# kserve/modelmesh

Hardware: AMD Instinct MI355X
Metric: placement decisions/sec at 100k models x 10k pods; p99 decision latency (higher is better)
Workload: dtype i64; 1 GPU; C3: 100000 models x 10000 pods, 8 load-target decision(s) per model per step = 800000 decisions per launch (SURVEY.md §8d synthetic fleet); streams=4, hw_queues=4, distinct_batches=6, issuers=1, library_submission_threads=0, resident_input_bytes=384000000

## Files before the change

modelmesh_amd/csrc/mmplace.hip:

```cpp
#include <hip/hip_runtime.h>
#include <dlfcn.h>
#include <rccl/rccl.h>
#include <rocprim/device/device_radix_sort.hpp>
#include <chrono>
#include <rocprim/device/device_merge_sort.hpp>
#include <rocprim/device/device_scan.hpp>

#include <algorithm>
#include <atomic>
#include <cstdarg>
#include <cstdio>
#include <cstdlib>
#include <cstring>
#include <map>
#include <memory>
#include <mutex>
#include <shared_mutex>
#include <thread>
#include <new>
#include <string>
#include <unordered_map>
#include <vector>

#include "../../include/mmplace.h"
// ... 21 lines not shown
    void *p = nullptr;
    size_t cap = 0;
    hipError_t ensure(size_t bytes)
    {
        if (bytes <= cap) return hipSuccess;
        if (p) (void)hipFree(p);
        p = nullptr;
        cap = 0;
        size_t want = std::max<size_t>(bytes, 256);
        want = (want + 255) & ~size_t(255);
        hipError_t e = hipMalloc(&p, want);
        if (e == hipSuccess) cap = want;
        return e;
    }
    void release()
    {
        if (p) (void)hipFree(p);
        p = nullptr;
        cap = 0;
    }
    template <class T>
    T *as() const { return reinterpret_cast<T *>(p); }
};

struct SnapBufs {
    DevBuf pods, lru, rem, cnt, rpm, orig, pos_of, elig, elig_nors, pref, has_pref, fullw, ge, pc, ph, nz, heads, bslots, bpm, bwin, bsurv, bpcs;
    DevBuf sel, rk;
    DevBuf amul;
    int32_t amul_w = 0;
    DevBuf memo, memo_cand, memo_rk;
    DevBuf lmemo;
    DevBuf ctpos;
    uint64_t types_gen = 0;
    int32_t n_bslots = 0;
    void release()
    {
        for (DevBuf *b : {&pods, &lru, &rem, &cnt, &rpm, &orig, &pos_of, &elig, &elig_nors, &pref, &has_pref, &fullw, &ge, &pc, &ph, &nz, &heads, &bslots, &bpm, &bwin, &bsurv, &bpcs, &ctpos, &sel, &rk, &amul, &memo, &memo_cand, &memo_rk, &lmemo})
            b->release();
    }
};

template <class SnapT>
SnapT snap_columns(const SnapBufs &B, int32_t P, int32_t W, int32_t T, bool any_rs, int64_t min_space)
{
    SnapT S{};
    S.P = P;
    S.W = W;
    S.T = T;
    S.any_rs = any_rs;
    S.min_space = min_space;
    S.lru = B.lru.as<int64_t>();
    S.rem = B.rem.as<int64_t>();
    S.cnt = B.cnt.as<int32_t>();
    S.rpm = B.rpm.as<int32_t>();
    S.orig = B.orig.as<int32_t>();
    S.pos_of = B.pos_of.as<int32_t>();
    S.elig = B.elig.as<uint64_t>();
    S.elig_nors = B.elig_nors.as<uint64_t>();
    S.pref = B.pref.as<uint64_t>();
    S.has_pref = B.has_pref.as<uint8_t>();
    S.fullw = B.fullw.as<uint64_t>();
    return S;
}

struct SnapSide {
    DevBuf d_allowed, d_has_allowed, stats_acc, d_pts, d_prohib, pstats, tstats, rmodels;
    DevBuf mtw;
    uint64_t types_gen = 0;
    bool rmodels_ok = false;
    std::vector<int32_t> pts_of;
    std::vector<uint64_t> pts_prohib;
    int32_t n_pts = 0, pts_tw = 1;
    std::vector<StatsAcc> pstats_h, tstats_h;
    void release()
    {
        for (DevBuf *b : {&d_allowed, &d_has_allowed, &stats_acc, &d_pts, &d_prohib, &pstats, &tstats, &rmodels, &mtw}) b->release();
    }
};

}

constexpr unsigned int kPinnedFlags = hipHostMallocCoherent | hipHostMallocMapped;
constexpr size_t kSelMaxBytes = (size_t)32 << 20;
constexpr int kTailStaticLds = 512;
constexpr int kTailBlocks = 16;
constexpr int kMaxMissBufs = 64;
constexpr int kFastSlots = 4;
constexpr int kFastN = 4096;
constexpr int kFastExtra = 16384;
struct FastSlot {
    std::mutex mu;
    hipStream_t stream = nullptr;
    mmp_place_req *reqs = nullptr;
    int32_t *extra = nullptr;
    mmp_place_out *outs = nullptr;
    uint32_t *done = nullptr;
    uint32_t *blocks = nullptr;
    std::atomic<uint32_t> seq{0};
};

struct Tuning {
    int32_t force_wave = 0;
    int32_t no_memo = 0;
    int32_t memo_from = -1;
    int32_t no_long_memo = 0;
    int32_t no_split = 0;
    int32_t split_from = -1;
    int32_t tail_blocks = kTailBlocks;
    int32_t split_notail = 0;
    int32_t no_long_lds = 0;
    int32_t no_caseb = 0;
    int32_t long_dense_from = kLongDenseFrom;
    bool long_dense_env = false;
    int32_t long_mode = -1;
    int32_t rank_mode = 0;
    int32_t no_delta = 0;
    int32_t plan_sorted = 0;
    int32_t plan_fused = 1;
    int32_t resident = 0;
};

struct mmp_ctx {
    mmp_config cfg{};
    hipStream_t stream = nullptr;
    std::mutex batch_mu, err_mu, cs_mu;
    std::shared_mutex mu;
    std::shared_ptr<struct IssuePool> pool;
    std::mutex pool_mu;
    struct Resident {
        std::atomic<bool> enabled{false}, running{false};
        std::atomic<uint32_t> generation{0};
        hipStream_t stream = nullptr;
        ResidentSlot *slots = nullptr;
        ResidentAnswer *answers = nullptr;
        ResidentCtl *ctl = nullptr;
        std::mutex launch_mu;
        std::mutex slot_mu[kResidentSlots];
        uint32_t seq[kResidentSlots] = {};
        std::atomic<uint32_t> rr{0};
        long long idle_ticks = 5'000'000;
        std::atomic<uint64_t> launches{0}, served{0}, punted{0};
        std::atomic<int> slow{0};
        std::atomic<int> punt_streak{0}, skip{0};
    } res;
    std::vector<hipStream_t> caller_streams;
    std::string err;
    FastSlot fast[kFastSlots];
    std::atomic<uint32_t> fast_rr{0};
    bool prof = false, prof_armed = false;
    hipEvent_t pe0 = nullptr, pe1 = nullptr;
    double last_kernel_ms = -1.0;
    size_t lds_limit = 64 * 1024;
    DevBuf rt_sreqs, rt_souts, rt_cnt;
    hipEvent_t reg_event = nullptr;
    std::atomic<bool> reg_pending{false};
    std::atomic<size_t> lds_granted{48 * 1024};
    Tuning tune;
    int32_t plan_grid_max = 0;
    struct MissBuf {
        std::mutex mu;
        bool used = false;
        hipStream_t st = nullptr;
        int32_t *words = nullptr;
        size_t cap = 0;
        int32_t *report = nullptr;
    };
    MissBuf miss_bufs[kMaxMissBufs];
// ... 348 lines not shown
    A.extra = static_cast<const int32_t *>(d_extra);
    A.outs = static_cast<mmp_place_out *>(d_outs);
    A.n = n;
    A.n_models = c->n_models;
    A.now = now;
    A.n_pods_all = n_pods_all;
    return A;
}

struct PlaceCall {
    const mmp_place_caller *caller = nullptr;
    int32_t extra_bound = 0;
    uint32_t *done_flag = nullptr;
    uint32_t done_seq = 0;
    uint32_t *done_blocks = nullptr;
    const mmp_place_req *inline_req = nullptr;
    const PlaceSegs *segs = nullptr;
    int32_t seg_blocks = 0;
    const GateArgs *fused_gate = nullptr;
    const mmp_gate_req *fused_greq = nullptr;
};

PlaceCall slot_call(FastSlot *f, const mmp_place_req *inline_req)
{
    PlaceCall o;
    o.done_flag = f->done;
    o.done_seq = ++f->seq;
    o.done_blocks = f->blocks;
    o.inline_req = inline_req;
    return o;
}

enum class PlaceRoute {
    memo_split, memo_split_c,
    multi, multi_m, multi_long, multi_long4,
    miss_single, single_lean, flag,
    batch, batch_m, batch_c, batch_c_m, batch_long, batch_long4, batch_long_c, batch_long4_c,
};
bool is_split(PlaceRoute r) { return r == PlaceRoute::memo_split || r == PlaceRoute::memo_split_c; }

struct RouteState {
    bool snap_long = false, snap_full = false;
    bool memo = false, lmemo = false;
    bool wins = false, rmodels = false;
    bool split_ok = false;
    bool memo_tail_lds = false;
};

bool long_first(const RouteState &s) { return s.snap_long && s.snap_full && s.rmodels; }

int32_t dense_from(const Tuning &t, const RouteState &s)
{
    return (long_first(s) && s.lmemo && !t.long_dense_env) ? INT32_MAX : t.long_dense_from;
}

PlaceRoute place_route(const Tuning &t, const RouteState &s, int32_t n, const PlaceCall &o)
{
    const bool caller = o.caller != nullptr, latency = o.inline_req || o.done_flag;
    const bool use_memo = !latency && !s.snap_long && !t.no_memo && !t.force_wave && s.wins && s.rmodels && s.memo &&
                          n >= (t.memo_from >= 0 ? t.memo_from : (caller ? kMemoFromC : kMemoFrom));
    const bool split = !o.segs && !t.no_split && s.split_ok;
    if (use_memo && split && s.memo_tail_lds && n >= (t.split_from >= 0 ? t.split_from : (caller ? kSplitFromC : kSplitFrom)))
        return caller ? PlaceRoute::memo_split_c : PlaceRoute::memo_split;
    if (o.segs) {
        if (s.snap_long) return n >= t.long_dense_from ? PlaceRoute::multi_long4 : PlaceRoute::multi_long;
        return use_memo ? PlaceRoute::multi_m : PlaceRoute::multi;
    }
    if (o.inline_req) return o.fused_gate ? PlaceRoute::miss_single : PlaceRoute::single_lean;
    if (o.done_flag && n > kPlaceBlock) return PlaceRoute::flag;
    if (caller && s.snap_long) return n >= dense_from(t, s) ? PlaceRoute::batch_long4_c : PlaceRoute::batch_long_c;
    if (use_memo) return caller ? PlaceRoute::batch_c_m : PlaceRoute::batch_m;
    if (caller) return PlaceRoute::batch_c;
    if (s.snap_long) return n >= dense_from(t, s) ? PlaceRoute::batch_long4 : PlaceRoute::batch_long;
    return PlaceRoute::batch;
}

template <class K>
const void *kfn(K *k) { return reinterpret_cast<const void *>(k); }
int grant_place_lds(mmp_ctx *c)
{
    static std::mutex grant_mu;
    std::lock_guard<std::mutex> g(grant_mu);
    const int want = (int)(c->lds_limit - kPlaceStaticLds);
    const int tail = want - kTailStaticLds;
    const struct {
        const void *fn;
        int max_lds;
    } kernels[] = {
        {kfn(place_batch_kernel), want}, {kfn(place_batch_m_kernel), want}, {kfn(place_batch_c_kernel), want},
        {kfn(place_batch_c_m_kernel), want}, {kfn(place_batch_long_kernel), want}, {kfn(place_batch_long4_kernel), want},
        {kfn(place_batch_long_c_kernel), want}, {kfn(place_batch_long4_c_kernel), want}, {kfn(place_batch_flag_kernel), want},
        {kfn(place_single_lean_kernel), want}, {kfn(miss_single_kernel), want}, {kfn(place_multi_kernel), want},
        {kfn(place_multi_m_kernel), want}, {kfn(place_multi_long_kernel), want}, {kfn(place_multi_long4_kernel), want},
        {kfn(place_tail_kernel), tail}, {kfn(place_tail_c_kernel), tail},
    };
    for (const auto &k : kernels) HIP_TRY(c, hipFuncSetAttribute(k.fn, hipFuncAttributeMaxDynamicSharedMemorySize, k.max_lds));
    c->lds_granted.store((size_t)want, std::memory_order_release);
    return MMP_OK;
}

int place_launch(mmp_ctx *c, const void *d_reqs, int32_t n, const void *d_extra, int64_t now, void *d_outs, hipStream_t st,
                 const PlaceCall &o = PlaceCall{})
{
    if (n == 0) return MMP_OK;
    if (o.caller && (o.segs || o.inline_req || o.done_flag)) return fail(c, MMP_EINVAL, "the single-caller form takes the batch kernels only");
    const Tuning &t = c->tune;
    const Snap &S = c->snap;
    const SnapBufs &B = c->sb[c->cur];
    PlaceArgs A = place_args(c, d_reqs, n, d_extra, now, d_outs, true, S.P);
    A.mtw = cur_side(c).rmodels_ok ? cur_side(c).mtw.as<int32_t>() : nullptr;
    A.wins = c->n_shards > 0 ? nullptr : B.heads.as<TypeWin>();
    A.force_wave = t.force_wave;
    A.done_flag = o.done_flag;
    A.done_seq = o.done_seq;
    A.extra_bound = o.extra_bound;
    RouteState rs;
    rs.snap_long = c->snap_long, rs.snap_full = c->snap_full, rs.memo = S.memo != nullptr, rs.lmemo = S.lmemo != nullptr;
    rs.wins = A.wins != nullptr, rs.rmodels = A.rmodels != nullptr;
    const bool latency = o.inline_req || o.done_flag;
    const int wpad = (S.W + 1) & ~1;
    size_t lds = std::max<size_t>((size_t)kPlaceWaves * 2 * wpad * sizeof(uint64_t), (size_t)place_lane_lds(S.T));
    A.long_first = long_first(rs) ? 1 : 0;
    if (A.long_first && !latency && !t.no_long_lds && n >= dense_from(t, rs)) {
        const size_t tb = long_tables_bytes(S.T, S.W);
        if (tb <= 24 * 1024 && ((lds + 15) & ~(size_t)15) + tb + kPlaceStaticLds <= c->lds_limit) {
            const size_t off = (lds + 15) & ~(size_t)15;
            A.long_first = 1 + (int32_t)off;
            lds = off + tb;
        }
    }
    if (c->snap_long && !latency && A.wins && !t.no_caseb && B.n_bslots > 0) {
        A.bslots = B.bslots.as<BSlot>();
        A.n_bslots = std::min(B.n_bslots, kBSlots);
        A.bwin = B.bwin.as<BLaunch>();
        A.bsurv = B.bsurv.as<uint64_t>();
        A.bpcs = B.bpcs.as<int32_t>();
    }
    if (lds + kPlaceStaticLds > c->lds_limit)
        return fail(c, MMP_EINVAL, "instance table too large for the LDS staging tile (%d pods: %zu + %d bytes of LDS, the device "
                    "gives a workgroup %zu)", S.P, lds, kPlaceStaticLds, c->lds_limit);
    if (lds > c->lds_granted.load(std::memory_order_acquire))
        if (const int rc = grant_place_lds(c)) return rc;
    const size_t lds_nobar = (size_t)kPlaceWaves * place_wave_lds(wpad);
    rs.memo_tail_lds = lds + kPlaceStaticLds + kTailStaticLds <= c->lds_limit;
    HIP_TRY(c, order_after_registry(c, st));
    const int grid = div_up(n, kPlaceBlock);
    const int cap = rest_list_cap(grid * kPlaceWaves);
    int32_t *words = nullptr, *report = nullptr;
    std::unique_lock<std::mutex> pair;
    rs.split_ok = !c->split_off.load(std::memory_order_relaxed);
    PlaceRoute r = place_route(t, rs, n, o);
    if (is_split(r) && (!miss_buffer(c, st, rest_buffer_ints(grid * kPlaceWaves), &words, &report, pair) ||
                        c->split_off.load(std::memory_order_relaxed))) {
        if (pair) pair.unlock();
        rs.split_ok = false;
        r = place_route(t, rs, n, o);
    }
    if (t.split_notail) words = nullptr;
    const size_t lds_memo = (size_t)kPlaceWaves * memo_stage_bytes(S.T);
    const dim3 block(kPlaceBlock), tails(t.tail_blocks);
    const bool tail = !t.split_notail;
    const mmp_place_caller C = o.caller ? *o.caller : mmp_place_caller{};
    switch (r) {
    case PlaceRoute::memo_split:
        hipLaunchKernelGGL(place_memo_kernel, dim3(grid), block, lds_memo, st, S, A, words, cap);
        if (tail) hipLaunchKernelGGL(place_tail_kernel, tails, block, lds, st, S, A, wpad, words, cap, report);
        break;
    case PlaceRoute::memo_split_c:
        hipLaunchKernelGGL(place_memo_c_kernel, dim3(grid), block, lds_memo, st, S, A, words, cap, C);
        if (tail) hipLaunchKernelGGL(place_tail_c_kernel, tails, block, lds, st, S, A, wpad, words, cap, report, C);
        break;
    case PlaceRoute::multi: hipLaunchKernelGGL(place_multi_kernel, dim3(o.seg_blocks), block, lds, st, S, A, wpad, *o.segs); break;
    case PlaceRoute::multi_m: hipLaunchKernelGGL(place_multi_m_kernel, dim3(o.seg_blocks), block, lds_nobar, st, S, A, wpad, *o.segs); break;
    case PlaceRoute::multi_long: hipLaunchKernelGGL(place_multi_long_kernel, dim3(o.seg_blocks), block, lds, st, S, A, wpad, *o.segs); break;
    case PlaceRoute::multi_long4: hipLaunchKernelGGL(place_multi_long4_kernel, dim3(o.seg_blocks), block, lds, st, S, A, wpad, *o.segs); break;
    case PlaceRoute::miss_single:
        hipLaunchKernelGGL(miss_single_kernel, dim3(1), dim3(128), lds, st, S, A, wpad, *o.inline_req, *o.fused_gate, *o.fused_greq);
        break;
    case PlaceRoute::single_lean: hipLaunchKernelGGL(place_single_lean_kernel, dim3(1), dim3(64), lds, st, S, A, wpad, *o.inline_req); break;
    case PlaceRoute::flag: hipLaunchKernelGGL(place_batch_flag_kernel, dim3(grid), block, lds, st, S, A, wpad, o.done_blocks); break;
    case PlaceRoute::batch: hipLaunchKernelGGL(place_batch_kernel, dim3(grid), block, lds, st, S, A, wpad); break;
    case PlaceRoute::batch_m: hipLaunchKernelGGL(place_batch_m_kernel, dim3(grid), block, lds_nobar, st, S, A, wpad); break;
    case PlaceRoute::batch_c: hipLaunchKernelGGL(place_batch_c_kernel, dim3(grid), block, lds, st, S, A, wpad, C); break;
    case PlaceRoute::batch_c_m: hipLaunchKernelGGL(place_batch_c_m_kernel, dim3(grid), block, lds_nobar, st, S, A, wpad, C); break;
    case PlaceRoute::batch_long: hipLaunchKernelGGL(place_batch_long_kernel, dim3(grid), block, lds_nobar, st, S, A, wpad); break;
    case PlaceRoute::batch_long4: hipLaunchKernelGGL(place_batch_long4_kernel, dim3(grid), block, lds, st, S, A, wpad); break;
    case PlaceRoute::batch_long_c: hipLaunchKernelGGL(place_batch_long_c_kernel, dim3(grid), block, lds_nobar, st, S, A, wpad, C); break;
    case PlaceRoute::batch_long4_c: hipLaunchKernelGGL(place_batch_long4_c_kernel, dim3(grid), block, lds, st, S, A, wpad, C); break;
    }
    HIP_TRY(c, hipGetLastError());
    if (is_split(r)) c->n_split.fetch_add(1, std::memory_order_relaxed);
    return MMP_OK;
}

}

extern "C" {

int mmp_abi_version(void) { return MMP_ABI_VERSION; }

int64_t mmp_min_space_units(int32_t dflt, int32_t threads, int64_t cap_units, int have_unload)
{
    const int32_t mn = (int32_t)((uint32_t)dflt * ((have_unload || threads <= 1) ? 1u : 2u));
    const int32_t a = (int32_t)((uint32_t)dflt * (uint32_t)threads);
    const int32_t b = (int32_t)(cap_units / 20);
    const int32_t target = a < b ? a : b;
    return mn > target ? mn : target;
}

int mmp_create(const mmp_config *cfg, mmp_ctx **out)
{
    if (!cfg || !out) return fail(nullptr, MMP_EINVAL, "mmp_create: null argument");
    *out = nullptr;
    int ndev = 0;
    hipError_t e = hipGetDeviceCount(&ndev);
    if (e != hipSuccess || ndev <= 0)
        return fail(nullptr, MMP_ENODEVICE, "no HIP device available (%s); libmmplace has no CPU path",
                    e == hipSuccess ? "device count 0" : hipGetErrorString(e));
    if (cfg->device < 0 || cfg->device >= ndev)
        return fail(nullptr, MMP_EINVAL, "device %d out of range (have %d)", cfg->device, ndev);
    if ((e = hipSetDevice(cfg->device)) != hipSuccess)
        return fail(nullptr, MMP_EHIP, "hipSetDevice: %s", hipGetErrorString(e));
    mmp_ctx *c = new (std::nothrow) mmp_ctx();
    if (!c) return fail(nullptr, MMP_ENOMEM, "out of memory");
    c->cfg = *cfg;
    {
        int v = 0;
        if (hipDeviceGetAttribute(&v, hipDeviceAttributeMaxSharedMemoryPerBlock, cfg->device) == hipSuccess && v > 0) c->lds_limit = (size_t)v;
    }
    c->tune = read_tuning();
    {
        int cus = 0, per_cu = 0;
        if (hipDeviceGetAttribute(&cus, hipDeviceAttributeMultiprocessorCount, cfg->device) == hipSuccess && cus > 0 &&
            hipFuncSetAttribute(reinterpret_cast<const void *>(proactive_plan_fused_kernel), hipFuncAttributeMaxDynamicSharedMemorySize,
                                (int)kPlanFusedLds) == hipSuccess &&
            hipOccupancyMaxActiveBlocksPerMultiprocessor(&per_cu, proactive_plan_fused_kernel, kPlanFusedBlock, kPlanFusedLds) == hipSuccess &&
            per_cu > 0)
            c->plan_grid_max = std::min(cus, kPlanFusedGrid);
        (void)hipGetLastError();
    }
    if ((e = hipStreamCreateWithFlags(&c->stream, hipStreamNonBlocking)) != hipSuccess) {
        delete c;
        return fail(nullptr, MMP_EHIP, "hipStreamCreate: %s", hipGetErrorString(e));
    }
    if ((e = hipEventCreateWithFlags(&c->reg_event, hipEventDisableTiming)) != hipSuccess) {
        (void)hipStreamDestroy(c->stream);
        delete c;
        return fail(nullptr, MMP_EHIP, "hipEventCreate: %s", hipGetErrorString(e));
    }
    for (FastSlot &f : c->fast) {
        int lo = 0, hi = 0;
        (void)hipDeviceGetStreamPriorityRange(&lo, &hi);
        hipError_t e1 = hipStreamCreateWithPriority(&f.stream, hipStreamNonBlocking, hi);
// ... 3961 lines not shown
```

modelmesh_amd/csrc/place_kernel.hpp:

```cpp
#pragma once
#include "snapshot.hpp"

namespace mmp {

#ifndef MMP_PLACE_WAVES
#define MMP_PLACE_WAVES 4
#endif
constexpr int kPlaceWaves = MMP_PLACE_WAVES;
constexpr int kPlaceBlock = kPlaceWaves * 64;

#ifdef MMP_PHASE_CLOCK
__device__ unsigned int g_phase[4096][16];
#define PHASE_ROW() (((blockIdx.x * (blockDim.x >> 6)) + (threadIdx.x >> 6)) & 4095)
#define PHASE_T0() unsigned long long ph_t_ = __builtin_amdgcn_s_memtime()
#define PHASE(k)                                                                                   \
    do {                                                                                           \
        const unsigned long long t_ = __builtin_amdgcn_s_memtime();                                \
        if (lane_id() == __ffsll((unsigned long long)__ballot(1)) - 1) g_phase[PHASE_ROW()][k] = (unsigned int)(t_ - ph_t_); \
        ph_t_ = t_;                                                                                \
    } while (0)
#define PHASE_COUNT(k, n)                                                                          \
    do {                                                                                           \
        if (lane_id() == __ffsll((unsigned long long)__ballot(1)) - 1) g_phase[PHASE_ROW()][k] += (unsigned int)(n); \
    } while (0)
// ... 2392 lines not shown
            const int rho_s = null_s ? 1 + srk - g0 : 0;
            bool self_pending = null_s;
            int t = index + (null0 ? 1 : 0);
#pragma unroll
            for (int i = 0; i < kInlineExcl; i++) {
                if (self_pending && selfpos < sx[i]) {
                    if (rho_s <= t) t++;
                    self_pending = false;
                }
                if ((xmask >> i) & 1u) {
                    if (1 + rkx[i] - g0 <= t) t++;
                }
            }
            if (self_pending && rho_s <= t) t++;
            cpos = t == 0 ? bestpos : SEL[g0 + t - 1];
        }
    }
    o.n_candidates = ccount;
    o.hash = (uint32_t)(hsum ^ (hsum >> 32)) ^ ((uint32_t)remaining * 0x9E3779B1u);
    if (cpos != kNoPos) {
        o.chosen = S.orig[cpos];
        if (!favour && cpos == selfpos) o.chosen = MMP_SELF;
    }
    return true;
}

__device__ __forceinline__ void build_long_memo_body(int t, const Snap &S, LongMemo *__restrict__ out)
{
    __shared__ LongCap caps[2 * kLongLevels];
    const int lane = lane_id();
    if (lane < 2 * kLongLevels) {
        const int level = lane >> 1;
        PlaceArgs A{};
        ResolvedReq r{};
        r.type = t;
        r.selfpos = -1;
        r.n_late = -1;
#pragma unroll
        for (int i = 0; i < kInlineExcl; i++) r.excl_pos[i] = -1;
#pragma unroll
        for (int i = 0; i < kLateExtra; i++) r.late_pos[i] = -1;
        bool bad = false;
        int p = -1;
        const uint64_t *E = S.elig + (size_t)t * S.W;
#pragma unroll
        for (int j = 0; j < kLongLevels - 1; j++) {
            if (j < level && !bad) {
                bool far = false;
                const int q = lane_first([&](int w) { return E[w]; }, p + 1, S.P, far, S.nz, (size_t)t * (size_t)(S.W + 1));
                if (far || q == kNoPos)
                    bad = true;
                else {
                    r.excl_pos[j] = q;
                    p = q;
                }
            }
        }
        r.n_excl = level;
        LongCap lc{};
        lc.nsb = lane & 1;
        if (!bad) {
            mmp_place_out o;
            const int code = lane_decide_r<false, true>(S, A, r, o, BLds{}, &lc);
            if (code != kLaneDone) lc.ok = 0;
        }
        caps[lane] = lc;
    }
    __syncthreads();
    if (lane < kLongLevels) {
        const LongCap &c0 = caps[2 * lane], &c1 = caps[2 * lane + 1];
        LongMemo M = (c0.ok ? c0 : c1).m;
        M.v[0] = c0.ok ? c0.m.v[0] : LongVar{};
        M.v[1] = c1.ok ? c1.m.v[1] : LongVar{};
        if (!c0.ok && !c1.ok) {
            M = LongMemo{};
            M.best0 = M.bestpos = kNoPos;
        }
        out[(size_t)t * kLongLevels + lane] = M;
    }
}

template <bool WITH_LONG, int FORM = kReq64, bool MEMO = false, bool NOBAR = false, bool LIST = false>
__device__ __forceinline__ void place_block(const Snap &S, const PlaceArgs &A, int32_t wpad, unsigned char *smem,
                                            uint32_t *done_blocks = nullptr, const mmp_place_caller &C = mmp_place_caller{}, int d_list = -1)
{
    static_assert(!(LIST && NOBAR), "the list form keeps the workgroup's barriers");
    __shared__ int32_t fb_list[kPlaceBlock], lr_list[kPlaceBlock];
    __shared__ int32_t fb_n, lr_n;
    TypeWin *s_wins = reinterpret_cast<TypeWin *>(smem);
    const int wave_nb = __builtin_amdgcn_readfirstlane((int)(threadIdx.x >> 6));
    unsigned char *smem_w = smem + (size_t)wave_nb * place_wave_lds(wpad);
    uint64_t *s_scr = NOBAR ? reinterpret_cast<uint64_t *>(smem_w)
                            : reinterpret_cast<uint64_t *>(smem + win_lds_bytes(S.T));
    if (threadIdx.x == 0) fb_n = lr_n = 0;
    const int d = LIST ? d_list : (int)(blockIdx.x * kPlaceBlock + threadIdx.x);
    PHASE_T0();
    PHASE_ABS(14);
    const bool use_wins = A.wins != nullptr;
    const TypeWin *Ws = NOBAR ? A.wins : s_wins;
    constexpr int kWinBytes = (int)sizeof(TypeWin);
    if (use_wins && !NOBAR) {
        const int wave = __builtin_amdgcn_readfirstlane((int)(threadIdx.x >> 6));
        const int chunks = ((S.T < kWinLds ? S.T : kWinLds) * kWinBytes + 1023) >> 10;
        const char *src = reinterpret_cast<const char *>(A.wins);
        char *dst = reinterpret_cast<char *>(s_wins);
        for (int c = wave; c < chunks; c += kPlaceWaves)
            __builtin_amdgcn_global_load_lds(src + (size_t)c * 1024 + lane_id() * 16,
                                             (__attribute__((address_space(3))) void *)(dst + c * 1024), 16, 0, 0);
    }
    bool live = LIST ? d >= 0 : d < A.n;
    mmp_place_req rq{};
    if (live) rq = fetch_req<FORM>(A, C, d);
    if (A.extra_bound != 0) {
        if (live && bad_extra_range(A, rq)) {
            live = false;
            mmp_place_out bo;
            bo.chosen = MMP_NONE;
            bo.best = MMP_BAD_REQUEST;
            bo.n_candidates = 0;
            bo.hash = 0;
            A.outs[d] = bo;
        }
    }
    Snap Sl = S;
    if (WITH_LONG && !NOBAR && A.long_first > 1) {
        unsigned char *tb = smem + (A.long_first - 1);
        const int nE = S.T * S.W, nPC = 2 * S.T * (S.W + 1);
        uint64_t *lE = reinterpret_cast<uint64_t *>(tb), *lP = lE + nE;
        int32_t *lpc = reinterpret_cast<int32_t *>(lP + nE), *lnz = lpc + nPC;
        for (int i = threadIdx.x; i < nE; i += kPlaceBlock) {
            lE[i] = S.elig[i];
            lP[i] = S.pref[i];
        }
        for (int i = threadIdx.x; i < nPC; i += kPlaceBlock) {
            lpc[i] = S.pc[i];
            lnz[i] = S.nz[i];
        }
        Sl.elig = lE;
        Sl.pref = lP;
        Sl.pc = lpc;
        Sl.nz = lnz;
    }
    BLds Bt{};
    if (WITH_LONG && A.n_bslots > 0) {
        Bt.slots = A.bslots;
        Bt.n_slots = A.n_bslots < kBSlots ? A.n_bslots : kBSlots;
        Bt.W = S.W;
        Bt.surv = A.bsurv;
        Bt.pcs = A.bpcs;
        Bt.launch = A.bwin;
    }
    if (!NOBAR) {
        asm volatile("s_waitcnt vmcnt(0)" ::: "memory");
        __syncthreads();
    }
    if (MEMO && live && memo_try<FORM>(S, A, rq, d, S.memo)) live = false;
    ResolvedReq r;
    int wcode = 0;
    if (live) r = resolve_req<false, true>(S, A, rq);
    PHASE(0);
    if (live) {
        mmp_place_out o;
        int code = kLaneHeadMiss;
        if (WITH_LONG && A.long_first) {
            merge_late_extras(r);
            const bool rec = S.lmemo != nullptr && long_memo_try(S, A, r, o);
            code = kLaneDone;
            if (!rec) code = lane_decide_r<false, true>(Sl, A, r, o, Bt);
        } else {
            if (use_wins)
                code = NOBAR ? lane_decide_win<false, false, 64>(S, A, r, Ws, s_scr + lane_id(), o)
                             : lane_decide_win(S, A, r, Ws, s_scr + threadIdx.x, o);
            if (code == kLaneHeadMiss) {
                merge_late_extras(r);
                code = lane_decide_r<false>(S, A, r, o, Bt);
            }
        }
        if (WITH_LONG && NOBAR && (code == kLaneLong || code == kLaneCaseB)) {
            code = lane_decide<false, true, FORM>(Sl, A, d, o, Bt, C);
            if (code == kLaneDone)
                store_out_streaming(A.outs + d, o);
            else
                wcode = 1;
        } else if (WITH_LONG && (code == kLaneLong || code == kLaneCaseB))
            lr_list[atomicAdd(&lr_n, 1)] = d;
        else if (code != kLaneDone) {
            if (NOBAR)
                wcode = 1;
            else
                fb_list[atomicAdd(&fb_n, 1)] = d;
        } else
            store_out_streaming(A.outs + d, o);
    }
    PHASE(8);
    if (NOBAR) {
        const uint64_t fb = __ballot(wcode != 0);
        if (fb) {
            const int wave = __builtin_amdgcn_readfirstlane((int)(threadIdx.x >> 6));
            int32_t *mine = fb_list + wave * 64;
            if (wcode) mine[__popcll((unsigned long long)(fb & ((1ull << lane_id()) - 1ull)))] = d;
            wave_sync();
            uint64_t *ew = reinterpret_cast<uint64_t *>(smem_w);
            uint64_t *fw = ew + wpad;
            const int nf = __popcll((unsigned long long)fb);
            for (int i = 0; i < nf; i++) {
                const int fd = __builtin_amdgcn_readfirstlane(mine[i]);
                place_one<FORM>(S, A, fd, ew, fw, C);
                wave_sync();
            }
        }
        PHASE(10);
        PHASE_COUNT(11, 1);
        PHASE_ABS(15);
        announce_done(DoneFlag{A.done_flag, done_blocks, A.done_seq});
        return;
    }
    __syncthreads();
    PHASE(9);
    if (WITH_LONG && lr_n != 0) {
        const int nlr = lr_n;
        if ((int)threadIdx.x < nlr) {
            const int ld = lr_list[threadIdx.x];
            mmp_place_out o;
            if (lane_decide<false, true, FORM>(Sl, A, ld, o, Bt, C) != kLaneDone)
                fb_list[atomicAdd(&fb_n, 1)] = ld;
            else
                store_out_streaming(A.outs + ld, o);
        }
        __syncthreads();
    }
    const int nfb = fb_n;
    if (nfb != 0) {
        const int wave = __builtin_amdgcn_readfirstlane((int)(threadIdx.x >> 6));
        uint64_t *ew = reinterpret_cast<uint64_t *>(smem) + (size_t)wave * 2 * wpad;
        uint64_t *fw = ew + wpad;
        for (int i = wave; i < nfb; i += kPlaceWaves) {
            const int fd = __builtin_amdgcn_readfirstlane(fb_list[i]);
            place_one<FORM>(S, A, fd, ew, fw, C);
            wave_sync();
            PHASE_COUNT(12, 1);
        }
    }
    PHASE(10);
    PHASE_COUNT(11, 1);
    PHASE_ABS(15);
    announce_done(DoneFlag{A.done_flag, done_blocks, A.done_seq});
    if (LIST) __syncthreads();
}

#ifndef MMP_PLACE_EU
#define MMP_PLACE_EU 6
#endif
__global__ __launch_bounds__(kPlaceBlock) __attribute__((amdgpu_waves_per_eu(MMP_PLACE_EU, MMP_PLACE_EU))) void place_batch_kernel(Snap S, PlaceArgs A, int32_t wpad)
{
    extern __shared__ __attribute__((aligned(16))) unsigned char smem[];
    place_block<false>(S, A, wpad, smem);
}

__global__ __launch_bounds__(kPlaceBlock) void place_batch_long_kernel(Snap S, PlaceArgs A, int32_t wpad)
{
    extern __shared__ __attribute__((aligned(16))) unsigned char smem[];
    place_block<true, kReq64, false, true>(S, A, wpad, smem);
}

constexpr int kLongDenseFrom = 3 * 4 * 256 * 64;
__global__ __launch_bounds__(kPlaceBlock) __attribute__((amdgpu_waves_per_eu(4, 4))) void place_batch_long4_kernel(Snap S, PlaceArgs A, int32_t wpad)
{
    extern __shared__ __attribute__((aligned(16))) unsigned char smem[];
    place_block<true>(S, A, wpad, smem);
}

#ifndef MMP_C_WAVES
#define MMP_C_WAVES 7
#endif
__global__ __launch_bounds__(kPlaceBlock) __attribute__((amdgpu_waves_per_eu(MMP_C_WAVES, MMP_C_WAVES))) void place_batch_c_kernel(Snap S, PlaceArgs A, int32_t wpad,
                                                                                                            mmp_place_caller C)
{
    extern __shared__ __attribute__((aligned(16))) unsigned char smem[];
    place_block<false, kReqC>(S, A, wpad, smem, nullptr, C);
}
__device__ __forceinline__ void build_memo_body(int t, const Snap &S, const TypeWin *__restrict__ wins, TypeMemo *__restrict__ memo,
                                                int32_t *__restrict__ cand, int16_t *__restrict__ rkt)
{
    constexpr int kScr = 2;
    __shared__ uint64_t scr[kWinWords * kScr];
    __shared__ MemoCap caps[2];
    __shared__ int ok[2];
    const int lane = lane_id();
    if (lane < 2) {
        PlaceArgs A{};
        ResolvedReq r{};
        r.type = t;
        r.selfpos = -1;
        r.n_late = -1;
#pragma unroll
        for (int i = 0; i < kInlineExcl; i++) r.excl_pos[i] = -1;
#pragma unroll
        for (int i = 0; i < kLateExtra; i++) r.late_pos[i] = -1;
        MemoCap mc{};
        mc.nsb = lane;
        mmp_place_out o;
        const int code = lane_decide_win<false, true, kScr>(S, A, r, wins, scr + lane, o, &mc);
        caps[lane] = mc;
        ok[lane] = code == kLaneDone && mc.ccount <= kMemoCand;
    }
    __syncthreads();
    const int w0 = wins[t].w0;
    const bool any = ok[0] || ok[1];
    const MemoCap &c0 = caps[ok[0] ? 0 : 1];
    if (lane == 0) {
        TypeMemoHead M{};
        M.b_rem = c0.b_rem;
        M.b_lru = c0.b_lru;
        M.best_is_full = c0.best_is_full;
        M.b_rpm = c0.b_rpm;
        M.best_idx = c0.best_idx;
        M.plain = c0.bestpos == c0.best0;
        M.w0 = w0;
        M.bestpos = c0.bestpos;
        M.best0 = c0.best0;
        M.e_rpm = c0.e_rpm;
        M.sbk = c0.sbk ? 1 : 0;
        M.end0 = caps[0].end;
        for (int v = 0; v < 2; v++) {
            const MemoCap &c = caps[v];
            M.v[v].valid = ok[v];
            M.v[v].lo = c.best0;
            M.v[v].hi = c.end == kNoPos ? S.P : c.end + 1;
            M.v[v].ccount = c.ccount;
            M.v[v].hsum = c.hsum;
            M.v[v].hash = (uint32_t)(c.hsum ^ (c.hsum >> 32));
        }
        static_cast<TypeMemoHead &>(memo[t]) = M;
    }
    __shared__ int32_t near_c[kMemoNear];
    __shared__ int32_t near_r[kMemoNear];
    near_c[lane] = 0;
    near_r[lane] = kRkNone;
    wave_sync();
    int32_t *out = cand + (size_t)t * kMemoCand;
    int16_t *rk = rkt + (size_t)t * kMemoCand;
    int running = 0;
    for (int j = 0; j < kWinWords; j++) {
        const int w = w0 + j, pos = w * 64 + lane;
        const uint64_t word = (ok[0] && w >= caps[0].wlo && w <= caps[0].whi) ? scr[j * kScr] : 0ull;
        const bool bit = (word >> lane) & 1ull;
        const int k = running + __popcll((unsigned long long)(word & ((1ull << lane) - 1ull)));
        int v = kRkNone;
        if (bit) {
            v = k;
            const int32_t pod = S.orig[pos];
            out[k] = pod;
            if (k < kMemoNear) near_c[k] = pod;
        }
        if (any && pos == c0.bestpos) v = 0;
        if (any && pos == c0.best0 && c0.best0 != c0.bestpos) v = kRkFirst;
        rk[j * 64 + lane] = (int16_t)v;
        if (any && pos >= c0.best0 && pos - c0.best0 < kMemoNear) near_r[pos - c0.best0] = v;
        running += __popcll((unsigned long long)word);
    }
    wave_sync();
    memo[t].cand64[lane] = near_c[lane];
    memo[t].rk64[lane] = (int16_t)near_r[lane];
}
__global__ __launch_bounds__(64) void build_sel_memo_kernel(Snap S, int32_t *__restrict__ sel, int32_t *__restrict__ rk, const TypeWin *__restrict__ wins,
                                                            TypeMemo *__restrict__ memo, int32_t *__restrict__ cand, int16_t *__restrict__ memo_rk,
                                                            LongMemo *__restrict__ lmemo)
{
    const int n_sel = sel ? 2 * S.T * S.W : 0;
    const int n_memo = S.T < kWinLds ? S.T : kWinLds;
    if ((int)blockIdx.x < n_sel)
        build_sel_body((int)blockIdx.x, S, sel, rk);
    else if ((int)blockIdx.x < n_sel + n_memo)
        build_memo_body((int)blockIdx.x - n_sel, S, wins, memo, cand, memo_rk);
    else
        build_long_memo_body((int)blockIdx.x - n_sel - n_memo, S, lmemo);
}

__global__ __launch_bounds__(kPlaceBlock) __attribute__((amdgpu_waves_per_eu(MMP_C_WAVES, MMP_C_WAVES))) void place_batch_c_m_kernel(Snap S, PlaceArgs A, int32_t wpad,
                                                                                                              mmp_place_caller C)
{
    extern __shared__ __attribute__((aligned(16))) unsigned char smem[];
    place_block<false, kReqC, true, true>(S, A, wpad, smem, nullptr, C);
}
__global__ __launch_bounds__(kPlaceBlock) __attribute__((amdgpu_waves_per_eu(7, 7))) void place_batch_m_kernel(Snap S, PlaceArgs A, int32_t wpad)
{
    extern __shared__ __attribute__((aligned(16))) unsigned char smem[];
    place_block<false, kReq64, true, true>(S, A, wpad, smem);
}
constexpr int kMemoFrom = 4 * 1024 * 64;
constexpr int kMemoFromC = 3 * 1024 * 64;
constexpr int kSplitFrom = 6 * 1024 * 64;
constexpr int kSplitFromC = 8 * 1024 * 64;

constexpr int kRestLists = 64;
constexpr int kRestCntStride = 32;
__host__ __device__ constexpr int rest_list_cap(int n_words) { return ((n_words + kRestLists - 1) / kRestLists) * 64; }
__host__ __device__ constexpr size_t rest_buffer_ints(int n_words) { return (size_t)kRestLists * kRestCntStride + (size_t)kRestLists * rest_list_cap(n_words); }

__device__ __forceinline__ void rest_append(int32_t *__restrict__ rest, int32_t cap, int d, bool todo)
{
    const uint64_t mk = __ballot(todo);
    if (mk && rest) {
        const int l = __builtin_amdgcn_readfirstlane(d >> 6) & (kRestLists - 1);
        const int first = __ffsll((unsigned long long)mk) - 1;
        int base = 0;
        if (lane_id() == first)
            base = __hip_atomic_fetch_add(rest + l * kRestCntStride, __popcll((unsigned long long)mk), __ATOMIC_RELAXED, __HIP_MEMORY_SCOPE_AGENT);
        base = readlane_i32(base, first);
        if (todo) rest[kRestLists * kRestCntStride + (size_t)l * cap + base + __popcll((unsigned long long)(mk & ((1ull << lane_id()) - 1ull)))] = d;
    }
}

template <int FORM>
__device__ __forceinline__ void place_memo_body(const Snap &S, const PlaceArgs &A, int32_t *__restrict__ rest, int32_t cap, const mmp_place_caller &C,
                                                unsigned char *smem)
{
    const int stage = memo_stage_bytes(S.T);
    unsigned char *mine = smem + (size_t)__builtin_amdgcn_readfirstlane((int)(threadIdx.x >> 6)) * stage;
    {
        const char *src = reinterpret_cast<const char *>(S.memo);
        for (int c = 0; c < stage; c += 1024)
            __builtin_amdgcn_global_load_lds(src + c + lane_id() * 16, (__attribute__((address_space(3))) void *)(mine + c), 16, 0, 0);
    }
    const int d = blockIdx.x * kPlaceBlock + threadIdx.x;
    bool live = d < A.n;
    mmp_place_req rq{};
    if (live) rq = fetch_req<FORM>(A, C, d);
    asm volatile("s_waitcnt vmcnt(0)" ::: "memory");
    wave_sync();
    if (A.extra_bound != 0) {
        if (live && bad_extra_range(A, rq)) {
            live = false;
            mmp_place_out bo;
            bo.chosen = MMP_NONE;
            bo.best = MMP_BAD_REQUEST;
            bo.n_candidates = 0;
            bo.hash = 0;
            A.outs[d] = bo;
        }
    }
    bool todo = false;
    if (live) todo = !memo_try<FORM>(S, A, rq, d, reinterpret_cast<const TypeMemo *>(mine));
    rest_append(rest, cap, d, todo);
}
__global__ __launch_bounds__(kPlaceBlock) __attribute__((amdgpu_waves_per_eu(8, 8))) void place_memo_kernel(Snap S, PlaceArgs A, int32_t *__restrict__ rest, int32_t cap)
{
    extern __shared__ __attribute__((aligned(16))) unsigned char smem[];
    place_memo_body<kReq64>(S, A, rest, cap, mmp_place_caller{}, smem);
}
__global__ __launch_bounds__(kPlaceBlock) __attribute__((amdgpu_waves_per_eu(8, 8))) void place_memo_c_kernel(Snap S, PlaceArgs A, int32_t *__restrict__ rest, int32_t cap,
                                                                                                           mmp_place_caller C)
{
    extern __shared__ __attribute__((aligned(16))) unsigned char smem[];
    place_memo_body<kReqC>(S, A, rest, cap, C, smem);
}

template <int FORM>
__device__ __forceinline__ void place_tail_body(const Snap &S, const PlaceArgs &A, int32_t wpad, unsigned char *smem, int32_t *__restrict__ rest, int32_t cap,
                                                int32_t *report, const mmp_place_caller &C)
{
    __shared__ int32_t t_cnt[kRestLists + 1];
    __builtin_amdgcn_s_setprio(3);
    PHASE_T0();
    const int tid = threadIdx.x;
    const int G = gridDim.x, g = blockIdx.x;
    if (g >= kRestLists) return;
    const int mine = (kRestLists - g + G - 1) / G;
    if (tid < 64) {
        const int c = tid < mine ? rest[(g + tid * G) * kRestCntStride] : 0;
        const int incl = wave_incl_scan_i32(c);
        t_cnt[tid + 1] = incl;
        if (tid == 0) t_cnt[0] = 0;
        if (report && g == 0) {
            const int all = wave_sum_i32(rest[tid * kRestCntStride]);
            if (tid == 0) {
                __hip_atomic_store(report, all, __ATOMIC_RELAXED, __HIP_MEMORY_SCOPE_SYSTEM);
                __hip_atomic_store(report + 1, A.n, __ATOMIC_RELAXED, __HIP_MEMORY_SCOPE_SYSTEM);
            }
        }
    }
    __syncthreads();
    const int total = t_cnt[mine];
    PHASE(13);
    for (int base = 0; base < total; base += kPlaceBlock) {
        int d = -1;
        const int i = base + tid;
        if (i < total) {
            int k = 0;
            while (t_cnt[k + 1] <= i) k++;
            d = rest[kRestLists * kRestCntStride + (size_t)(g + k * G) * cap + (i - t_cnt[k])];
        }
        PHASE(14);
        place_block<false, FORM, false, false, true>(S, A, wpad, smem, nullptr, C, d);
    }
    if (tid < mine) rest[(g + tid * G) * kRestCntStride] = 0;
}
#ifndef MMP_TAIL_EU
#define MMP_TAIL_EU 5
#endif
__global__ __launch_bounds__(kPlaceBlock) __attribute__((amdgpu_waves_per_eu(MMP_TAIL_EU, MMP_TAIL_EU))) void place_tail_kernel(Snap S, PlaceArgs A, int32_t wpad, int32_t *__restrict__ rest, int32_t cap, int32_t *report)
{
    extern __shared__ __attribute__((aligned(16))) unsigned char smem[];
    place_tail_body<kReq64>(S, A, wpad, smem, rest, cap, report, mmp_place_caller{});
}
__global__ __launch_bounds__(kPlaceBlock) __attribute__((amdgpu_waves_per_eu(MMP_TAIL_EU, MMP_TAIL_EU))) void place_tail_c_kernel(Snap S, PlaceArgs A, int32_t wpad, int32_t *__restrict__ rest, int32_t cap, int32_t *report,
                                                                   mmp_place_caller C)
{
    extern __shared__ __attribute__((aligned(16))) unsigned char smem[];
    place_tail_body<kReqC>(S, A, wpad, smem, rest, cap, report, C);
}

__global__ __launch_bounds__(kPlaceBlock) void place_batch_long_c_kernel(Snap S, PlaceArgs A, int32_t wpad, mmp_place_caller C)
{
    extern __shared__ __attribute__((aligned(16))) unsigned char smem[];
    place_block<true, kReqC, false, true>(S, A, wpad, smem, nullptr, C);
}
__global__ __launch_bounds__(kPlaceBlock) __attribute__((amdgpu_waves_per_eu(4, 4))) void place_batch_long4_c_kernel(Snap S, PlaceArgs A, int32_t wpad,
                                                                                                                  mmp_place_caller C)
{
    extern __shared__ __attribute__((aligned(16))) unsigned char smem[];
    place_block<true, kReqC>(S, A, wpad, smem, nullptr, C);
}

__global__ __launch_bounds__(kPlaceBlock) void place_batch_flag_kernel(Snap S, PlaceArgs A, int32_t wpad, uint32_t *done_blocks)
{
    extern __shared__ __attribute__((aligned(16))) unsigned char smem[];
    place_block<true>(S, A, wpad, smem, done_blocks);
}


constexpr int kResidentSlots = 64;
constexpr uint32_t kResidentPunt = 0x80000000u;
constexpr int kResidentNowBits = 44;
__device__ __forceinline__ void load16_sys(const void *p, uint64_t &lo, uint64_t &hi)
{
    typedef unsigned int u32x4_t __attribute__((ext_vector_type(4)));
    u32x4_t v;
    asm volatile("global_load_dwordx4 %0, %1, off sc0 sc1\n\ts_waitcnt vmcnt(0)" : "=v"(v) : "v"(p) : "memory");
    lo = ((uint64_t)v.y << 32) | v.x;
    hi = ((uint64_t)v.w << 32) | v.z;
}
struct __attribute__((aligned(16))) ResidentSlot {
    mmp_place_req req;
    uint64_t bell;
    uint64_t pad[7];
};
static_assert(sizeof(ResidentSlot) == 128, "ResidentSlot is 128 bytes");
struct __attribute__((aligned(64))) ResidentAnswer {
    mmp_place_out out;
    uint32_t done;
    uint32_t pad[11];
};
static_assert(sizeof(ResidentAnswer) == 64, "ResidentAnswer is 64 bytes");
struct ResidentCtl {
    uint32_t stop;
    uint32_t exited;
    uint32_t pad[14];
};

__global__ __launch_bounds__(64) void place_resident_kernel(Snap S, PlaceArgs A, ResidentSlot *slots, ResidentAnswer *answers,
                                                             ResidentCtl *ctl, long long idle_ticks, uint32_t generation)
{
    extern __shared__ __attribute__((aligned(16))) unsigned char smem[];
    TypeWin *s_wins = reinterpret_cast<TypeWin *>(smem);
    uint64_t *s_scr = reinterpret_cast<uint64_t *>(smem + kWinLdsBytes);
    const int lane = lane_id();
    const bool use_wins = A.wins != nullptr;
    if (use_wins) {
        const int chunks = ((S.T < kWinLds ? S.T : kWinLds) * (int)sizeof(TypeWin) + 1023) >> 10;
        const char *src = reinterpret_cast<const char *>(A.wins);
        char *dst = reinterpret_cast<char *>(s_wins);
        for (int c = 0; c < chunks; c++)
            __builtin_amdgcn_global_load_lds(src + (size_t)c * 1024 + lane * 16,
                                             (__attribute__((address_space(3))) void *)(dst + c * 1024), 16, 0, 0);
        asm volatile("s_waitcnt vmcnt(0)" ::: "memory");
    }
    wave_sync();
    ResidentSlot *slot = &slots[lane];
// ... 63 lines not shown
```

Baseline: 49.63 billion decisions/s.

## Store full request records in rest lists and drain them per wavefront

The memo pass now writes the whole request, vector-stored as 16-byte records, into the rest lists instead of only the decision index. The tail kernel then drains each list with one wavefront at a time, without workgroup barriers or an LDS prefix scan, and it uses the smaller per-wave LDS size. The report total is gathered with an agent-scope arrival counter instead of block 0 summing the counts. This is meant to avoid re-fetching requests in the tail and to avoid barrier stalls between waves. In exchange the rest buffer grows several-fold and the memo kernel does extra stores.

```diff
diff --git a/modelmesh_amd/csrc/mmplace.hip b/modelmesh_amd/csrc/mmplace.hip
--- a/modelmesh_amd/csrc/mmplace.hip
+++ b/modelmesh_amd/csrc/mmplace.hip
@@ -127,7 +127,6 @@
 
 constexpr unsigned int kPinnedFlags = hipHostMallocCoherent | hipHostMallocMapped;
 constexpr size_t kSelMaxBytes = (size_t)32 << 20;
-constexpr int kTailStaticLds = 512;
 constexpr int kTailBlocks = 16;
 constexpr int kMaxMissBufs = 64;
 constexpr int kFastSlots = 4;
@@ -642,7 +641,6 @@
     static std::mutex grant_mu;
     std::lock_guard<std::mutex> g(grant_mu);
     const int want = (int)(c->lds_limit - kPlaceStaticLds);
-    const int tail = want - kTailStaticLds;
     const struct {
         const void *fn;
         int max_lds;
@@ -652,7 +650,7 @@
         {kfn(place_batch_long_c_kernel), want}, {kfn(place_batch_long4_c_kernel), want}, {kfn(place_batch_flag_kernel), want},
         {kfn(place_single_lean_kernel), want}, {kfn(miss_single_kernel), want}, {kfn(place_multi_kernel), want},
         {kfn(place_multi_m_kernel), want}, {kfn(place_multi_long_kernel), want}, {kfn(place_multi_long4_kernel), want},
-        {kfn(place_tail_kernel), tail}, {kfn(place_tail_c_kernel), tail},
+        {kfn(place_tail_kernel), want}, {kfn(place_tail_c_kernel), want},
     };
     for (const auto &k : kernels) HIP_TRY(c, hipFuncSetAttribute(k.fn, hipFuncAttributeMaxDynamicSharedMemorySize, k.max_lds));
     c->lds_granted.store((size_t)want, std::memory_order_release);
@@ -702,7 +700,7 @@
     if (lds > c->lds_granted.load(std::memory_order_acquire))
         if (const int rc = grant_place_lds(c)) return rc;
     const size_t lds_nobar = (size_t)kPlaceWaves * place_wave_lds(wpad);
-    rs.memo_tail_lds = lds + kPlaceStaticLds + kTailStaticLds <= c->lds_limit;
+    rs.memo_tail_lds = lds_nobar + kPlaceStaticLds <= c->lds_limit;
     HIP_TRY(c, order_after_registry(c, st));
     const int grid = div_up(n, kPlaceBlock);
     const int cap = rest_list_cap(grid * kPlaceWaves);
@@ -710,7 +708,7 @@
     std::unique_lock<std::mutex> pair;
     rs.split_ok = !c->split_off.load(std::memory_order_relaxed);
     PlaceRoute r = place_route(t, rs, n, o);
-    if (is_split(r) && (!miss_buffer(c, st, rest_buffer_ints(grid * kPlaceWaves), &words, &report, pair) ||
+    if (is_split(r) && (!miss_buffer(c, st, rest_buffer_ints(grid * kPlaceWaves, o.caller ? kReqC : kReq64), &words, &report, pair) ||
                         c->split_off.load(std::memory_order_relaxed))) {
         if (pair) pair.unlock();
         rs.split_ok = false;
@@ -724,11 +722,11 @@
     switch (r) {
     case PlaceRoute::memo_split:
         hipLaunchKernelGGL(place_memo_kernel, dim3(grid), block, lds_memo, st, S, A, words, cap);
-        if (tail) hipLaunchKernelGGL(place_tail_kernel, tails, block, lds, st, S, A, wpad, words, cap, report);
+        if (tail) hipLaunchKernelGGL(place_tail_kernel, tails, block, lds_nobar, st, S, A, wpad, words, cap, report);
         break;
     case PlaceRoute::memo_split_c:
         hipLaunchKernelGGL(place_memo_c_kernel, dim3(grid), block, lds_memo, st, S, A, words, cap, C);
-        if (tail) hipLaunchKernelGGL(place_tail_c_kernel, tails, block, lds, st, S, A, wpad, words, cap, report, C);
+        if (tail) hipLaunchKernelGGL(place_tail_c_kernel, tails, block, lds_nobar, st, S, A, wpad, words, cap, report, C);
         break;
     case PlaceRoute::multi: hipLaunchKernelGGL(place_multi_kernel, dim3(o.seg_blocks), block, lds, st, S, A, wpad, *o.segs); break;
     case PlaceRoute::multi_m: hipLaunchKernelGGL(place_multi_m_kernel, dim3(o.seg_blocks), block, lds_nobar, st, S, A, wpad, *o.segs); break;
diff --git a/modelmesh_amd/csrc/place_kernel.hpp b/modelmesh_amd/csrc/place_kernel.hpp
--- a/modelmesh_amd/csrc/place_kernel.hpp
+++ b/modelmesh_amd/csrc/place_kernel.hpp
@@ -2498,9 +2498,10 @@
 
 template <bool WITH_LONG, int FORM = kReq64, bool MEMO = false, bool NOBAR = false, bool LIST = false>
 __device__ __forceinline__ void place_block(const Snap &S, const PlaceArgs &A, int32_t wpad, unsigned char *smem,
-                                            uint32_t *done_blocks = nullptr, const mmp_place_caller &C = mmp_place_caller{}, int d_list = -1)
-{
-    static_assert(!(LIST && NOBAR), "the list form keeps the workgroup's barriers");
+                                            uint32_t *done_blocks = nullptr, const mmp_place_caller &C = mmp_place_caller{}, int d_list = -1,
+                                            const mmp_place_req &rq_list = mmp_place_req{})
+{
+    static_assert(!LIST || NOBAR, "the list form is a wavefront on its own: no workgroup barrier");
     __shared__ int32_t fb_list[kPlaceBlock], lr_list[kPlaceBlock];
     __shared__ int32_t fb_n, lr_n;
     TypeWin *s_wins = reinterpret_cast<TypeWin *>(smem);
@@ -2526,7 +2527,10 @@
     }
     bool live = LIST ? d >= 0 : d < A.n;
     mmp_place_req rq{};
-    if (live) rq = fetch_req<FORM>(A, C, d);
+    if (LIST)
+        rq = rq_list;
+    else if (live)
+        rq = fetch_req<FORM>(A, C, d);
     if (A.extra_bound != 0) {
         if (live && bad_extra_range(A, rq)) {
             live = false;
@@ -2628,7 +2632,8 @@
         PHASE(10);
         PHASE_COUNT(11, 1);
         PHASE_ABS(15);
-        announce_done(DoneFlag{A.done_flag, done_blocks, A.done_seq});
+        if (!LIST) announce_done(DoneFlag{A.done_flag, done_blocks, A.done_seq});
+        if (LIST) wave_sync();
         return;
     }
     __syncthreads();
@@ -2661,7 +2666,6 @@
     PHASE_COUNT(11, 1);
     PHASE_ABS(15);
     announce_done(DoneFlag{A.done_flag, done_blocks, A.done_seq});
-    if (LIST) __syncthreads();
 }
 
 #ifndef MMP_PLACE_EU
@@ -2811,10 +2815,81 @@
 
 constexpr int kRestLists = 64;
 constexpr int kRestCntStride = 32;
+constexpr int kRestFirst = 16;
+template <int FORM>
+struct RestEntry;
+template <>
+struct __attribute__((aligned(16))) RestEntry<kReq64> {
+    mmp_place_req rq;
+    int32_t d, pad_[3];
+};
+template <>
+struct __attribute__((aligned(16))) RestEntry<kReqC> {
+    mmp_place_req_c rq;
+    int32_t d, pad_;
+};
+static_assert(sizeof(RestEntry<kReq64>) == 80 && sizeof(RestEntry<kReqC>) == 32, "records are whole 16-byte vectors");
+__host__ __device__ constexpr int rest_entry_bytes(int form) { return form == kReqC ? (int)sizeof(RestEntry<kReqC>) : (int)sizeof(RestEntry<kReq64>); }
 __host__ __device__ constexpr int rest_list_cap(int n_words) { return ((n_words + kRestLists - 1) / kRestLists) * 64; }
-__host__ __device__ constexpr size_t rest_buffer_ints(int n_words) { return (size_t)kRestLists * kRestCntStride + (size_t)kRestLists * rest_list_cap(n_words); }
-
-__device__ __forceinline__ void rest_append(int32_t *__restrict__ rest, int32_t cap, int d, bool todo)
+__host__ __device__ constexpr size_t rest_buffer_ints(int n_words, int form)
+{
+    return (size_t)kRestLists * kRestCntStride + (size_t)kRestLists * rest_list_cap(n_words) * (rest_entry_bytes(form) / 4);
+}
+template <int FORM>
+__device__ __forceinline__ RestEntry<FORM> *rest_list(int32_t *rest, int32_t cap, int l)
+{
+    return reinterpret_cast<RestEntry<FORM> *>(rest + kRestLists * kRestCntStride) + (size_t)l * cap;
+}
+template <class E>
+__device__ __forceinline__ void rest_entry_store(E *p, const E &e)
+{
+    typedef int v4i_ __attribute__((ext_vector_type(4)));
+    v4i_ v[sizeof(E) / 16];
+    __builtin_memcpy(v, &e, sizeof(E));
+#pragma unroll
+    for (int j = 0; j < (int)(sizeof(E) / 16); j++) reinterpret_cast<v4i_ *>(p)[j] = v[j];
+}
+template <class E>
+__device__ __forceinline__ E rest_entry_load(const E *p)
+{
+    typedef int v4i_ __attribute__((ext_vector_type(4)));
+    v4i_ v[sizeof(E) / 16];
+#pragma unroll
+    for (int j = 0; j < (int)(sizeof(E) / 16); j++) v[j] = reinterpret_cast<const v4i_ *>(p)[j];
+    E e;
+    __builtin_memcpy(&e, v, sizeof(E));
+    return e;
+}
+__device__ __forceinline__ void rest_entry_set(RestEntry<kReq64> &e, const mmp_place_req &rq) { e.rq = rq; }
+__device__ __forceinline__ void rest_entry_set(RestEntry<kReqC> &e, const mmp_place_req &rq)
+{
+    e.rq.model = rq.model;
+    e.rq.pick = rq.pick;
+    e.rq.last_used = rq.last_used;
+    e.rq.extra_off = rq.extra_off;
+    e.rq.n_extra = rq.n_extra;
+}
+__device__ __forceinline__ mmp_place_req rest_entry_req(const RestEntry<kReq64> &e, const mmp_place_caller &) { return e.rq; }
+__device__ __forceinline__ mmp_place_req rest_entry_req(const RestEntry<kReqC> &e, const mmp_place_caller &C)
+{
+    mmp_place_req r;
+    r.model = e.rq.model;
+    r.self_pod = C.self_pod;
+    r.flags = C.flags;
+    r.pick = e.rq.pick;
+    r.last_used = e.rq.last_used;
+    r.extra_off = e.rq.extra_off;
+    r.n_extra = e.rq.n_extra;
+    r.fresh_lru = C.fresh_lru;
+    r.fresh_capacity = C.fresh_capacity;
+    r.fresh_used = C.fresh_used;
+    r.fresh_count = C.fresh_count;
+    r.fresh_rpm = C.fresh_rpm;
+    return r;
+}
+
+template <int FORM>
+__device__ __forceinline__ void rest_append(int32_t *__restrict__ rest, int32_t cap, int d, bool todo, const PlaceArgs &A, const mmp_place_caller &C)
 {
     const uint64_t mk = __ballot(todo);
     if (mk && rest) {
@@ -2824,7 +2899,12 @@
         if (lane_id() == first)
             base = __hip_atomic_fetch_add(rest + l * kRestCntStride, __popcll((unsigned long long)mk), __ATOMIC_RELAXED, __HIP_MEMORY_SCOPE_AGENT);
         base = readlane_i32(base, first);
-        if (todo) rest[kRestLists * kRestCntStride + (size_t)l * cap + base + __popcll((unsigned long long)(mk & ((1ull << lane_id()) - 1ull)))] = d;
+        if (todo) {
+            RestEntry<FORM> e{};
+            rest_entry_set(e, fetch_req<FORM>(A, C, d));
+            e.d = d;
+            rest_entry_store(rest_list<FORM>(rest, cap, l) + base + __popcll((unsigned long long)(mk & ((1ull << lane_id()) - 1ull))), e);
+        }
     }
 }
 
@@ -2858,7 +2938,7 @@
     }
     bool todo = false;
     if (live) todo = !memo_try<FORM>(S, A, rq, d, reinterpret_cast<const TypeMemo *>(mine));
-    rest_append(rest, cap, d, todo);
+    rest_append<FORM>(rest, cap, d, todo, A, C);
 }
 __global__ __launch_bounds__(kPlaceBlock) __attribute__((amdgpu_waves_per_eu(8, 8))) void place_memo_kernel(Snap S, PlaceArgs A, int32_t *__restrict__ rest, int32_t cap)
 {
@@ -2876,41 +2956,40 @@
 __device__ __forceinline__ void place_tail_body(const Snap &S, const PlaceArgs &A, int32_t wpad, unsigned char *smem, int32_t *__restrict__ rest, int32_t cap,
                                                 int32_t *report, const mmp_place_caller &C)
 {
-    __shared__ int32_t t_cnt[kRestLists + 1];
     __builtin_amdgcn_s_setprio(3);
     PHASE_T0();
-    const int tid = threadIdx.x;
-    const int G = gridDim.x, g = blockIdx.x;
-    if (g >= kRestLists) return;
-    const int mine = (kRestLists - g + G - 1) / G;
-    if (tid < 64) {
-        const int c = tid < mine ? rest[(g + tid * G) * kRestCntStride] : 0;
-        const int incl = wave_incl_scan_i32(c);
-        t_cnt[tid + 1] = incl;
-        if (tid == 0) t_cnt[0] = 0;
-        if (report && g == 0) {
-            const int all = wave_sum_i32(rest[tid * kRestCntStride]);
-            if (tid == 0) {
-                __hip_atomic_store(report, all, __ATOMIC_RELAXED, __HIP_MEMORY_SCOPE_SYSTEM);
-                __hip_atomic_store(report + 1, A.n, __ATOMIC_RELAXED, __HIP_MEMORY_SCOPE_SYSTEM);
-            }
-        }
-    }
-    __syncthreads();
-    const int total = t_cnt[mine];
-    PHASE(13);
-    for (int base = 0; base < total; base += kPlaceBlock) {
-        int d = -1;
-        const int i = base + tid;
-        if (i < total) {
-            int k = 0;
-            while (t_cnt[k + 1] <= i) k++;
-            d = rest[kRestLists * kRestCntStride + (size_t)(g + k * G) * cap + (i - t_cnt[k])];
-        }
-        PHASE(14);
-        place_block<false, FORM, false, false, true>(S, A, wpad, smem, nullptr, C, d);
-    }
-    if (tid < mine) rest[(g + tid * G) * kRestCntStride] = 0;
+    const int lane = lane_id();
+    const int all = (int)gridDim.x * kPlaceWaves, nw = all < kRestLists ? all : kRestLists;
+    const int w = __builtin_amdgcn_readfirstlane((int)(blockIdx.x * kPlaceWaves + (threadIdx.x >> 6)));
+    if (w >= nw) return;
+    int mine = 0;
+    for (int l = w; l < kRestLists; l += nw) {
+        int32_t *cnt_p = rest + l * kRestCntStride;
+        const RestEntry<FORM> *list = rest_list<FORM>(rest, cap, l);
+        int cnt = *cnt_p;
+        RestEntry<FORM> e{};
+        if (lane < kRestFirst) e = rest_entry_load(list + lane);
+        cnt = __builtin_amdgcn_readfirstlane(cnt);
+        PHASE(13);
+        mine += cnt;
+        for (int base = 0; base < cnt; base = base ? base + 64 : kRestFirst) {
+            const int i = base + lane;
+            if (base != 0 && i < cnt) e = rest_entry_load(list + i);
+            const bool have = i < cnt && (base != 0 || lane < kRestFirst);
+            place_block<false, FORM, false, true, true>(S, A, wpad, smem, nullptr, C, have ? e.d : -1, rest_entry_req(e, C));
+        }
+        if (lane == 0 && cnt != 0) *cnt_p = 0;
+    }
+    if (report && lane == 0) {
+        unsigned long long *arrive = reinterpret_cast<unsigned long long *>(rest + 2);
+        const unsigned long long was =
+            __hip_atomic_fetch_add(arrive, (1ull << 32) | (unsigned long long)(uint32_t)mine, __ATOMIC_RELAXED, __HIP_MEMORY_SCOPE_AGENT);
+        if ((int)(was >> 32) == nw - 1) {
+            __hip_atomic_store(report, (int32_t)(uint32_t)was + mine, __ATOMIC_RELAXED, __HIP_MEMORY_SCOPE_SYSTEM);
+            __hip_atomic_store(report + 1, A.n, __ATOMIC_RELAXED, __HIP_MEMORY_SCOPE_SYSTEM);
+            __hip_atomic_store(arrive, 0ull, __ATOMIC_RELAXED, __HIP_MEMORY_SCOPE_AGENT);
+        }
+    }
 }
 #ifndef MMP_TAIL_EU
 #define MMP_TAIL_EU 5
```

New measurement: 45.62 billion decisions/s. 0.919x the previous value.
